# medivhna/TF_Face_Toolbox

Measured on NVIDIA B200. Metric: A-softmax head fwd+bwd samples/sec at C=85,742 D=512, 1/2/4/8 B200, higher is better.
Workload: dtype bf16

## Files before the change

### tf_face_toolbox_b200/csrc/asm_api.cu

```cuda
#include <math.h>
#include <stdio.h>
#include <stdlib.h>
#include <string.h>

#include <new>
#include <vector>

#include "../../include/asoftmax_b200.h"
#include "asm_kernels.cuh"

using namespace asmh;

struct asm_head {
  asm_config cfg;
  int device = 0;
  int num_sms = 148;
  int Cp = 0;
  int NT = 0;
  char* ws = nullptr;
  size_t ws_bytes = 0;
  Step st{};
  size_t dx_part_capacity = 0;
  UmmaMaps maps{};
  int maps_B = -1;
// ... 42 lines not shown
  if (c->D <= 0 || c->D % 16 != 0) return false;
  if (c->C_total <= 0 || c->C_local <= 0 || c->class_offset < 0) return false;
  if ((long long)c->class_offset + c->C_local > c->C_total) return false;
  if (c->B_max <= 0 || c->m < 1 || c->m > 4) return false;
  if (c->mode != ASM_MODE_FP32 && c->mode != ASM_MODE_BF16) return false;
  if (c->mode == ASM_MODE_BF16 && c->D % 64 != 0) return false;
  if (c->world < 1 || c->rank < 0 || c->rank >= c->world) return false;
  if (c->nccl_comm != nullptr) return false;
  return true;
}

bool use_x3(const asm_config& c) {
  if (c.mode != ASM_MODE_FP32 || c.D % 64 != 0) return false;
  const char* e = getenv("ASM_FP32_SIMT");
  return !(e && atoi(e) != 0);
}
bool use_tc(const asm_config& c) { return c.mode == ASM_MODE_BF16 || use_x3(c); }

Layout make_layout(const asm_config& c, int num_sms) {
  Layout L{};
  const bool tc = use_tc(c);
  const size_t planes = use_x3(c) ? 3 : 1;
  const size_t B = c.B_max, D = c.D;
  L.Cp = (int)align_up(c.C_local, 256);
  L.NT = (L.Cp + 127) / 128;
  if (L.NT < 2 * num_sms) L.NT = 2 * num_sms;
  L.MT = 2 * (int)((B + 127) / 128);
  if (L.MT < 4 * (int)((B + 255) / 256)) L.MT = 4 * (int)((B + 255) / 256);
  const int ks_simt = simt_dx_splits(c.B_max, c.D, L.Cp);
  const int ks_umma = umma_dx_splits(c.B_max, c.D, L.Cp, num_sms, 1);
  const int ks_one = tc ? umma_dx_splits(128, c.D, L.Cp, num_sms, 1)
                        : simt_dx_splits(128, c.D, L.Cp);
  const size_t cap_full = (size_t)(tc ? ks_umma : ks_simt) * B * D;
  const size_t cap_one = (size_t)ks_one * (B < 128 ? B : 128) * D;
  L.dx_capacity = cap_full > cap_one ? cap_full : cap_one;
  size_t off = 0;
  auto take = [&](size_t bytes) { size_t o = off; off = align_up(off + bytes, 256); return o; };
  L.ylocal = take(B * 4);
  L.flags = take(256);
  L.n = take(B * 4);
  L.inv_n = take(B * 4);
  L.inv_c = take((size_t)L.Cp * 4);
  L.margin = take(kMarginRecordFloats * 4);
  L.tgt_s = take(B * 4);
  L.tgt_f = take(B * 4);
  L.part = take(B * (size_t)L.NT * 8);
  L.stats_local = take(3 * B * 4);
  L.lse = take(B * 4);
  L.negoff = take(B * 4);
  L.gtarget = take(B * 4);
  L.rcoef = take(B * 4);
  L.rowloss = take(B * 4);
  L.counter = take(256);
  L.wsq_part = take(((size_t)L.Cp / 32 + 16) * 4);
  L.wsq_ticket = take(256);
  L.q_part = take((size_t)L.MT * L.Cp * 4);
  L.G = take(align_up(B, 64) * (size_t)L.Cp * (c.mode == ASM_MODE_BF16 ? 2 : 4));
  L.dx_part = take(L.dx_capacity * 4);
  if (tc) {
    L.Xb = take(planes * B * D * 2);
    L.Wb = take(planes * D * (size_t)L.Cp * 2);
  } else {
    L.Xs = take(B * D * 4);
  }
  if (c.world > 1) {
    L.Xg = take(B * D * 4);
    L.step_dev = take(256);
  }
  L.total = off;
  return L;
}

int fail(asm_head* h, int code, const char* fmt, const char* detail) {
  char* dst = h ? h->err : g_create_err;
  snprintf(dst, 512, fmt, detail ? detail : "");
  return code;
}

#define CU_TRY(h, expr)                                                         \
  do {                                                                          \
    cudaError_t e__ = (expr);                                                   \
    if (e__ != cudaSuccess) return fail(h, ASM_ERR_CUDA, #expr ": %s", cudaGetErrorString(e__)); \
  } while (0)

void mark(asm_head* h, const char* name, cudaStream_t stream, bool phase_start = true) {
  h->launches += 1;
  if (h->phase_profiling && !phase_start) return;
  if (h->profiling && h->n_marks < asm_head::kMaxMarks) {
    cudaEventRecord(h->ev[h->n_marks], stream);
    h->mark_name[h->n_marks] = name;
    h->n_marks += 1;
  }
}
void mark_end(asm_head* h, cudaStream_t stream) {
  if (h->profiling) cudaEventRecord(h->ev[h->n_marks], stream);
}

int check_launch(asm_head* h, const char* what) {
  cudaError_t e = cudaGetLastError();
  if (e != cudaSuccess) {
    snprintf(h->err, 512, "%s: %s", what, cudaGetErrorString(e));
    return ASM_ERR_CUDA;
  }
  return ASM_OK;
}

bool split_active(const asm_head* h) {
// ... 195 lines not shown
    return fail(nullptr, ASM_ERR_CUDA, "cudaGetDevice failed%s", "");
  cudaDeviceGetAttribute(&major, cudaDevAttrComputeCapabilityMajor, dev);
  cudaDeviceGetAttribute(&sms, cudaDevAttrMultiProcessorCount, dev);
  if (major != 10)
    return fail(nullptr, ASM_ERR_NO_DEVICE, "device is not sm_100 (Blackwell B200) %s", "");
  asm_head* h = new (std::nothrow) asm_head();
  if (!h) return fail(nullptr, ASM_ERR_ALLOC, "host allocation failed%s", "");
  h->cfg = *cfg;
  h->device = dev;
  h->num_sms = sms > 0 ? sms : 148;
  h->err[0] = 0;
  const char* e;
  if ((e = getenv("ASM_UMMA_MN_LBO"))) h->tune.mn_lbo = (uint32_t)atoi(e);
  if ((e = getenv("ASM_UMMA_MN_SBO"))) h->tune.mn_sbo = (uint32_t)atoi(e);
  if ((e = getenv("ASM_UMMA_MN_KSTEP"))) h->tune.mn_kstep = (uint32_t)atoi(e);
  if ((e = getenv("ASM_UMMA_DEBUG")) && atoi(e) != 0) {
#ifdef ASM_BRINGUP
    h->tune.debug_flags = (uint32_t)atoi(e);
#else
    delete h;
    return fail(nullptr, ASM_ERR_INVALID_ARG,
                "ASM_UMMA_DEBUG is set but this library was built without -DASM_BRINGUP%s", "");
#endif
  }
  if ((e = getenv("ASM_L2_ORDER"))) h->tune.l2_order = atoi(e) != 0;
  if ((e = getenv("ASM_DW_TMA"))) h->tune.dw_tma = atoi(e) != 0;
  if ((e = getenv("ASM_L2_HINTS"))) h->tune.l2_hints = (uint32_t)atoi(e);
  if ((e = getenv("ASM_UMMA_CG"))) h->tune.cg_mask = (uint32_t)atoi(e);
  if ((e = getenv("ASM_UMMA_BN"))) h->tune.bn = (uint32_t)atoi(e);
  if ((e = getenv("ASM_NO_OVERLAP")) && atoi(e)) h->overlap = false;
  h->dw_pairs = (h->num_sms / 2) * 42 / 74;
  if ((e = getenv("ASM_DW_PAIRS"))) h->dw_pairs = atoi(e);
  if (h->dw_pairs < 0 || h->dw_pairs >= h->num_sms / 2) h->dw_pairs = 0;
  if ((e = getenv("ASM_PDL"))) h->pdl = atoi(e) != 0;
  if ((e = getenv("ASM_DEFER_LOSS"))) h->defer_loss = atoi(e) != 0;
  if ((e = getenv("ASM_OPT_STREAM"))) h->opt_stream = atoi(e) != 0;
  if (cudaStreamCreateWithFlags(&h->side, cudaStreamNonBlocking) != cudaSuccess ||
      cudaEventCreateWithFlags(&h->ev_fork, cudaEventDisableTiming) != cudaSuccess ||
      cudaEventCreateWithFlags(&h->ev_join, cudaEventDisableTiming) != cudaSuccess) {
    cudaGetLastError();
    h->side = nullptr;
  }
  if ((e = getenv("ASM_L2_PERSIST_MB"))) h->l2_persist_bytes = (size_t)atoi(e) << 20;
  const Layout L = make_layout(*cfg, h->num_sms);
  cudaError_t ce = cudaMalloc(&h->ws, L.total);
  if (ce != cudaSuccess) {
    fail(nullptr, ASM_ERR_ALLOC, "cudaMalloc(workspace): %s", cudaGetErrorString(ce));
    delete h;
    return ASM_ERR_ALLOC;
  }
  h->ws_bytes = L.total;
  cudaMemset(h->ws, 0, L.total);
  h->tc = use_tc(*cfg);
  if (h->tc) {
    ce = umma_configure();
    if (ce != cudaSuccess) {
      fail(nullptr, ASM_ERR_CUDA, "cudaFuncSetAttribute(smem): %s", cudaGetErrorString(ce));
      cudaFree(h->ws);
      delete h;
      return ASM_ERR_CUDA;
    }
  }
  Step& s = h->st;
  s.D = cfg->D;
  s.C = cfg->C_local;
  s.Cp = L.Cp;
  s.C_total = cfg->C_total;
  s.class_offset = cfg->class_offset;
  s.m = cfg->m;
  s.mode = cfg->mode;
  s.x3 = use_x3(*cfg) ? 1 : 0;
  char* w = h->ws;
  s.ylocal = (int*)(w + L.ylocal);
  s.flags = (int*)(w + L.flags);
  s.n = (float*)(w + L.n);
  s.inv_n = (float*)(w + L.inv_n);
  s.inv_c = (float*)(w + L.inv_c);
  s.tgt_s = (float*)(w + L.tgt_s);
  s.tgt_f = (float*)(w + L.tgt_f);
  s.part = (float2*)(w + L.part);
  s.stats_local = (float*)(w + L.stats_local);
  s.lse = (float*)(w + L.lse);
  s.negoff = (float*)(w + L.negoff);
  s.gtarget = (float*)(w + L.gtarget);
  s.rcoef = (float*)(w + L.rcoef);
  s.rowloss = (float*)(w + L.rowloss);
  s.counter = (unsigned int*)(w + L.counter);
  s.q_part = (float*)(w + L.q_part);
  s.wsq_part = (float*)(w + L.wsq_part);
  s.wsq_ticket = (unsigned int*)(w + L.wsq_ticket);
  s.gscale = 1.0f;
  s.wd_g = 0.0f;
  s.reg_scale = 0.0f;
  s.reg_out = nullptr;
  s.G = (void*)(w + L.G);
  s.dx_part = (float*)(w + L.dx_part);
  h->dx_part_capacity = L.dx_capacity;
  if (h->tc) {
    s.Xb = (__nv_bfloat16*)(w + L.Xb);
    s.Wb = (__nv_bfloat16*)(w + L.Wb);
  } else {
    s.Xs = (float*)(w + L.Xs);
  }
  s.mg.kind = 0;
  if (cfg->world > 1) {
    h->Xg = (float*)(w + L.Xg);
// ... 290 lines not shown
```

### tf_face_toolbox_b200/csrc/asm_kernels.cuh

```cuda
#pragma once
#include <cuda.h>
#include <cuda_bf16.h>
#include <cuda_runtime.h>
#include <stdint.h>

#include "asm_common.cuh"

namespace asmh {

struct OptParams {
  int kind;
  float lr;
  float mu, b1, b2, eps, wd;
};
__host__ __device__ inline void opt_apply(const OptParams& o, float grad, float& w, float& s0,
                                          float& s1) {
  const float g = grad + o.wd * w;
  if (o.kind == 1) {
    s0 = o.mu * s0 + g;
    w -= o.lr * s0;
  } else {
    s0 = o.b1 * s0 + (1.0f - o.b1) * g;
    s1 = o.b2 * s1 + (1.0f - o.b2) * g * g;
#ifdef __CUDA_ARCH__
// ... 71 lines not shown
  int B, D, C, Cp, C_total, class_offset, m, mode;
  float lambda, invB;
  const float* lambda_dev;
  float gscale;
  float wd_g;
  float reg_scale;
  float* reg_out;
  float* wsq_part;
  unsigned int* wsq_ticket;
  const float* X;
  int x_bf16;
  const float* W;
  float* logits;
  float* dX;
  float* dW;
  float* loss;
  int* ylocal;
  int* flags;
  float* n;
  float* inv_n;
  float* inv_c;
  float* tgt_s;
  float* tgt_f;
  float2* part;
  int NT;
  float* stats_local;
  float* lse;
  float* negoff;
  float* gtarget;
  float* rcoef;
  float* rowloss;
  unsigned int* counter;
  float* q_part;
  int MT;
  void* G;
  int Bp;
  float* dx_part;
  int KS;
  __nv_bfloat16* Xb;
  __nv_bfloat16* Wb;
  int x3;
  OptParams opt;
  float* Wmut;
  float* opt_s0;
  float* opt_s1;
  int l2_hints;
  int pdl;
  int defer_loss;
  Margin mg;
  float* Xs;
};

void launch_prep(const Step& s, const void* labels, int label_bytes, cudaStream_t st, const P2P* p = nullptr);
void launch_combine_p2p(const Step& s, const P2P& p, cudaStream_t st);
void launch_dx_finish_p2p(const Step& s, const P2P& p, cudaStream_t st);
void launch_combine_local(const Step& s, cudaStream_t st);
void launch_combine_global(const Step& s, const float* stats_all, int n_shards, cudaStream_t st);
void launch_combine_fused(const Step& s, cudaStream_t st);
void launch_dx_finish(const Step& s, cudaStream_t st);
void launch_opt_stream(const Step& s, const float* dW, cudaStream_t st);

void p2p_preload_kernels();
void prep_preload_kernels();
void simt_preload_kernels();

void launch_simt_forward(const Step& s, cudaStream_t st);
void launch_simt_bwdg(const Step& s, cudaStream_t st);
void launch_simt_dw(const Step& s, cudaStream_t st);
void launch_simt_dx(const Step& s, cudaStream_t st);
int simt_forward_tiles(int C);
int simt_dx_splits(int B, int D, int Cp);

struct UmmaMaps {
  CUtensorMap xb_k, xb_k256, xb_mn, wb_mn, wb_mn32, wb_k, wb_k128, g_k, g_mn, g_st, g_st32, wb_box;
  CUtensorMap dw_even, dw_odd;
  CUtensorMap dx_st;
  int dx_ok;
  const void* dw_ptr;
  int dw_ok;
};
struct UmmaTuning {
  uint32_t mn_lbo, mn_sbo, mn_kstep;
  uint32_t cg_mask;
  uint32_t debug_flags;
  uint32_t bn;
  uint32_t l2_order;
  uint32_t dw_tma;
  uint32_t side_by_side;
  uint32_t l2_hints;
};
struct UmmaArgs {
  int mt, nt, ks, kb_total, kb_per;
  int nseg, kb_seg;
  int segA[6], segB[6];
  uint64_t desc_hi_k, desc_hi_mn;
  uint32_t kstep_mn;
  uint32_t debug_flags;
  int rev;
  int kstride;
  int dw_tma;
  int dx_tma;
  int dw_shift;
  int store_evict_first;
};
cudaError_t umma_configure();
bool umma_build_maps(UmmaMaps* m, const Step& s);
// ... 17 lines not shown
```

### tf_face_toolbox_b200/csrc/asm_prep.cu

```cuda
#include <stdlib.h>

#include "asm_common.cuh"
#include "asm_kernels.cuh"
#include "asm_p2p.cuh"
#include "asm_rows.cuh"

namespace asmh {

__device__ __forceinline__ void prep_row_tail(const Step& s, int row, float acc, long long y) {
  const float nn = sqrtf(acc);
  s.n[row] = nn;
  s.inv_n[row] = nn > 0.f ? 1.0f / nn : 0.f;
  const long long yl = y - s.class_offset;
  s.ylocal[row] = (y < 0 || y >= s.C_total) ? -2 : ((yl >= 0 && yl < s.C) ? (int)yl : -1);
  s.tgt_s[row] = 0.f;
  s.tgt_f[row] = 0.f;
}

template <int PL>
__device__ __forceinline__ void prep_row_scaled(const Step& s, const char* x, char* xg, int esz, bool gather,
                                                int row, long long y) {
  const int tx = threadIdx.x & 31;
  const float4* x4 = reinterpret_cast<const float4*>(x);
  const int n16 = s.D * esz / 16;
  const int epp = 16 / esz;
  auto sq16 = [&](const float4& v) {
    if (esz == 2) {
      const __nv_bfloat162* h2 = reinterpret_cast<const __nv_bfloat162*>(&v);
      float a = 0.f;
#pragma unroll
      for (int q = 0; q < 4; ++q) {
        const float l = __low2float(h2[q]), h = __high2float(h2[q]);
        a = fmaf(l, l, a);
        a = fmaf(h, h, a);
      }
      return a;
    }
    return fmaf(v.x, v.x, fmaf(v.y, v.y, fmaf(v.z, v.z, v.w * v.w)));
  };
  float4 v[4];
  float acc = 0.f;
  for (int i0 = 0; i0 < n16; i0 += 128) {
#pragma unroll
    for (int u = 0; u < 4; ++u) {
      const int i = i0 + u * 32 + tx;
      v[u] = i < n16 ? (gather ? __ldcv(x4 + i) : __ldg(x4 + i)) : make_float4(0.f, 0.f, 0.f, 0.f);
    }
#pragma unroll
    for (int u = 0; u < 4; ++u) {
      const int i = i0 + u * 32 + tx;
      if (i < n16) {
        if (gather) reinterpret_cast<float4*>(xg)[i] = v[u];
        acc += sq16(v[u]);
      }
    }
  }
  acc = warp_sum(acc);
  const float nn = sqrtf(acc);
  const float sc = nn > 0.f ? s.mg.s / nn : 0.f;
  auto put = [&](int d, float e) {
    const float u = e * sc;
    if (PL > 0) {
      __nv_bfloat16* dst = s.Xb + (size_t)row * PL * s.D + d;
      float r = u;
#pragma unroll
      for (int p2 = 0; p2 < PL; ++p2) {
        const __nv_bfloat16 hv = __float2bfloat16_rn(r);
        dst[(size_t)p2 * s.D] = hv;
        r -= __bfloat162float(hv);
      }
    } else {
      s.Xs[(size_t)row * s.D + d] = u;
    }
  };
  auto put16 = [&](int e0, const float4& w) {
    if (esz == 2) {
      const __nv_bfloat162* h2 = reinterpret_cast<const __nv_bfloat162*>(&w);
#pragma unroll
      for (int q = 0; q < 4; ++q) {
        put(e0 + 2 * q, __low2float(h2[q]));
        put(e0 + 2 * q + 1, __high2float(h2[q]));
      }
    } else {
      put(e0, w.x); put(e0 + 1, w.y); put(e0 + 2, w.z); put(e0 + 3, w.w);
    }
  };
  const float4* again = gather ? reinterpret_cast<const float4*>(xg) : x4;
  for (int i0 = 0; i0 < n16; i0 += 128) {
#pragma unroll
    for (int u = 0; u < 4; ++u) {
      const int i = i0 + u * 32 + tx;
      if (i < n16) put16(i * epp, n16 <= 128 ? v[u] : again[i]);
    }
  }
  if (tx == 0) prep_row_tail(s, row, acc, y);
}

template <bool VEC2, int PL, int TX, int TY, int U, bool ADD>
__device__ __forceinline__ void prep_block(const Step& s, const void* labels, int label_bytes,
                                           int nwb, int npub, const P2P& p, const int vblock,
                                           float (*red)[2 * TX]) {
  static_assert(TX * TY == 256, "256 threads");
  const int tid = threadIdx.x;
  if (vblock < npub) {
    const unsigned cur = p2p_current_step(p);
    float4* xs = reinterpret_cast<float4*>(p.x(p.rank, cur & 1));
    int* ys = p.y(p.rank, cur & 1);
    const size_t n4 = (size_t)p.b_local * p.D * (s.x_bf16 ? 2 : 4) / 16;
    for (size_t i = vblock * (size_t)256 + tid; i < n4; i += (size_t)npub * 256)
      xs[i] = __ldg(reinterpret_cast<const float4*>(p.x_local) + i);
    for (int i = vblock * 256 + tid; i < p.b_local; i += npub * 256)
      ys[i] = p.y_bytes == 8 ? (int)reinterpret_cast<const long long*>(p.y_local)[i]
                             : reinterpret_cast<const int*>(p.y_local)[i];
    if (block_ticket(p.tickets + 0, (unsigned)npub) == (unsigned)npub - 1 && tid == 0)
      p2p_publish(p, 0, cur);
    return;
  }
  const int bid = vblock - npub;
  if (bid < nwb) {
    const int tx = tid % TX, ty = tid / TX;
    const int j0 = (bid * TX + tx) * 2;
    float a0 = 0.f, a1 = 0.f;
    if (j0 < s.Cp) {
      const bool v0 = j0 < s.C, v1 = j0 + 1 < s.C;
      const float* w = s.W + j0;
      constexpr bool BF16 = PL > 0;
      __nv_bfloat16* wb = BF16 ? s.Wb + (size_t)(j0 >> 6) * s.D * 64 + (j0 & 63) : nullptr;
      const size_t plane = (size_t)s.D * s.Cp;
      for (int d0 = ty; d0 < s.D; d0 += TY * U) {
        float x0[U], x1[U];
#pragma unroll
        for (int u = 0; u < U; ++u) {
          const int d = d0 + TY * u;
          x0[u] = 0.f; x1[u] = 0.f;
          if (d < s.D) {
            if (VEC2) {
              if (v1) {
                const float2* wp = reinterpret_cast<const float2*>(w + (size_t)d * s.C);
                const float2 v = s.l2_hints ? __ldcs(wp) : __ldg(wp);
                x0[u] = v.x; x1[u] = v.y;
              } else if (v0) {
                x0[u] = __ldg(w + (size_t)d * s.C);
              }
            } else {
              if (v0) x0[u] = __ldg(w + (size_t)d * s.C);
              if (v1) x1[u] = __ldg(w + (size_t)d * s.C + 1);
            }
          }
        }
#pragma unroll
        for (int u = 0; u < U; ++u) {
          const int d = d0 + TY * u;
          a0 = fmaf(x0[u], x0[u], a0);
          a1 = fmaf(x1[u], x1[u], a1);
          if (BF16 && d < s.D) {
            __nv_bfloat162* dst = reinterpret_cast<__nv_bfloat162*>(wb + (size_t)d * 64);
            float r0 = x0[u], r1 = x1[u];
#pragma unroll
            for (int p = 0; p < PL; ++p) {
              const __nv_bfloat162 hv = __floats2bfloat162_rn(r0, r1);
              dst[(size_t)p * (plane / 2)] = hv;
              r0 -= __low2float(hv);
              r1 -= __high2float(hv);
            }
          }
        }
      }
    }
    red[ty][tx * 2] = a0;
    red[ty][tx * 2 + 1] = a1;
    __syncthreads();
    for (int t = tid; t < 2 * TX; t += 256) {
      float acc = 0.f;
#pragma unroll
      for (int r = 0; r < TY; ++r) acc += red[r][t];
      const int j = bid * 2 * TX + t;
      if (j < s.Cp) s.inv_c[j] = (j < s.C && acc > 0.f) ? rsqrtf(acc) : 0.f;
      if (s.reg_out) red[0][t] = j < s.C ? acc : 0.f;
    }
    if (s.reg_out) {
      __syncthreads();
      if (tid == 0) {
        float tot = 0.f;
        for (int t = 0; t < 2 * TX; ++t) tot += red[0][t];
        s.wsq_part[bid] = tot;
      }
      if (block_ticket(s.wsq_ticket, (unsigned)nwb) == (unsigned)nwb - 1) {
        __shared__ float wred[256];
        float acc = 0.f;
        for (int i = tid; i < nwb; i += 256) acc += __ldcg(s.wsq_part + i);
        wred[tid] = acc;
        __syncthreads();
        for (int o = 128; o > 0; o >>= 1) {
          if (tid < o) wred[tid] += wred[tid + o];
          __syncthreads();
        }
        if (tid == 0) *s.reg_out = s.reg_scale * wred[0];
      }
    }
  } else {
    const int tx = tid & 31;
    const int row = (bid - nwb) * 8 + (tid >> 5);
    if (row >= s.B) return;
    const int esz = s.x_bf16 ? 2 : 4;
    const char* x = reinterpret_cast<const char*>(s.X) + (size_t)row * s.D * esz;
    char* xg = nullptr;
    long long y;
    if (npub > 0) {
      const unsigned cur = p2p_current_step(p);
      const int src = row / p.b_local, lr = row - src * p.b_local;
      if (tx == 0) p2p_wait(p, 0, src, cur);
      __syncwarp();
      x = reinterpret_cast<const char*>(p.x(src, cur & 1)) + (size_t)lr * s.D * esz;
      xg = reinterpret_cast<char*>(p.Xg) + (size_t)row * s.D * esz;
      y = (long long)__ldcv(p.y(src, cur & 1) + lr);
    } else {
      y = label_bytes == 8 ? reinterpret_cast<const long long*>(labels)[row]
                           : (long long)reinterpret_cast<const int*>(labels)[row];
    }
    if (ADD) {
      prep_row_scaled<PL>(s, x, xg, esz, npub > 0, row, y);
      return;
    }
    float acc = 0.f;
    auto emit = [&](int d, float v) {
      acc = fmaf(v, v, acc);
      if (PL > 0) {
        __nv_bfloat16* dst = s.Xb + (size_t)row * PL * s.D + d;
        float r = v;
#pragma unroll
        for (int p2 = 0; p2 < PL; ++p2) {
          const __nv_bfloat16 hv = __float2bfloat16_rn(r);
          dst[(size_t)p2 * s.D] = hv;
          r -= __bfloat162float(hv);
        }
      }
    };
    auto emit16 = [&](int e0, const float4& v) {
      if (s.x_bf16) {
        const __nv_bfloat162* h2 = reinterpret_cast<const __nv_bfloat162*>(&v);
#pragma unroll
        for (int q = 0; q < 4; ++q) {
          emit(e0 + 2 * q, __low2float(h2[q]));
          emit(e0 + 2 * q + 1, __high2float(h2[q]));
        }
      } else {
        emit(e0, v.x); emit(e0 + 1, v.y); emit(e0 + 2, v.z); emit(e0 + 3, v.w);
      }
    };
    {
      const float4* x4 = reinterpret_cast<const float4*>(x);
      const int n16 = s.D * esz / 16;
      const int epp = 16 / esz;
      for (int i0 = 0; i0 < n16; i0 += 128) {
        float4 v[4];
#pragma unroll
        for (int u = 0; u < 4; ++u) {
          const int i = i0 + u * 32 + tx;
          v[u] = i < n16 ? (npub > 0 ? __ldcv(x4 + i) : __ldg(x4 + i)) : make_float4(0.f, 0.f, 0.f, 0.f);
        }
#pragma unroll
        for (int u = 0; u < 4; ++u) {
          const int i = i0 + u * 32 + tx;
          if (i < n16) {
            if (npub > 0) reinterpret_cast<float4*>(xg)[i] = v[u];
            emit16(i * epp, v[u]);
          }
        }
      }
    }
    acc = warp_sum(acc);
    if (tx == 0) prep_row_tail(s, row, acc, y);
  }
}

template <bool VEC2, int PL, int TX, int TY, int U, bool ADD>
__global__ void __launch_bounds__(256) prep_kernel(Step s, const void* labels, int label_bytes,
                                                   int nwb, int npub, P2P p) {
  pdl_trigger();
  __shared__ float red[TY][2 * TX];
  if (blockIdx.x == 0 && threadIdx.x == 0) *const_cast<Margin*>(margin_record(s.tgt_s)) = s.mg;
  prep_block<VEC2, PL, TX, TY, U, ADD>(s, labels, label_bytes, nwb, npub, p, (int)blockIdx.x, red);
}

template <int TX, int TY, int U, bool ADD>
static void launch_prep_t(const Step& s, const void* labels, int label_bytes, cudaStream_t st, const P2P* p) {
  const int nwb = (s.Cp + 2 * TX - 1) / (2 * TX);
  const int nxb = (s.B + 7) / 8;
  int npub = 0;
  P2P pp{};
  if (p != nullptr && p->world > 1) {
    pp = *p;
    npub = (int)(((size_t)p->b_local * p->D / 4 + 2047) / 2048);
    if (npub < 1) npub = 1;
    if (npub > 32) npub = 32;
  }
  const bool vec2 = (s.C % 2 == 0) && ((reinterpret_cast<uintptr_t>(s.W) & 7) == 0);
  dim3 grd(npub + nwb + nxb);
  if (s.x3) {
    if (vec2) prep_kernel<true, 3, TX, TY, U, ADD><<<grd, 256, 0, st>>>(s, labels, label_bytes, nwb, npub, pp);
    else prep_kernel<false, 3, TX, TY, U, ADD><<<grd, 256, 0, st>>>(s, labels, label_bytes, nwb, npub, pp);
  } else if (s.mode == 1) {
    if (vec2) prep_kernel<true, 1, TX, TY, U, ADD><<<grd, 256, 0, st>>>(s, labels, label_bytes, nwb, npub, pp);
    else prep_kernel<false, 1, TX, TY, U, ADD><<<grd, 256, 0, st>>>(s, labels, label_bytes, nwb, npub, pp);
  } else {
    if (vec2) prep_kernel<true, 0, TX, TY, U, ADD><<<grd, 256, 0, st>>>(s, labels, label_bytes, nwb, npub, pp);
    else prep_kernel<false, 0, TX, TY, U, ADD><<<grd, 256, 0, st>>>(s, labels, label_bytes, nwb, npub, pp);
  }
}

template <int TX, int TY, int U>
static void launch_prep_t(const Step& s, const void* labels, int label_bytes, cudaStream_t st, const P2P* p) {
  if (s.mg.kind != 0) launch_prep_t<TX, TY, U, true>(s, labels, label_bytes, st, p);
  else launch_prep_t<TX, TY, U, false>(s, labels, label_bytes, st, p);
}

void launch_prep(const Step& s, const void* labels, int label_bytes, cudaStream_t st, const P2P* p) {
  static int shape = -1, small_auto = -1;
  if (shape < 0) {
    const char* e = getenv("ASM_PREP_SHAPE");
    shape = e ? atoi(e) : 0;
    e = getenv("ASM_PREP_AUTO");
    small_auto = (e && atoi(e) != 0) ? 1 : 0;
  }
  if (shape == 0 && small_auto && s.Cp <= 32768) {
    launch_prep_t<16, 16, 8>(s, labels, label_bytes, st, p);
    return;
  }
  if (shape == 1) launch_prep_t<32, 8, 16>(s, labels, label_bytes, st, p);
  else if (shape == 2) launch_prep_t<16, 16, 8>(s, labels, label_bytes, st, p);
  else if (shape == 3) launch_prep_t<128, 2, 16>(s, labels, label_bytes, st, p);
  else launch_prep_t<32, 8, 4>(s, labels, label_bytes, st, p);
}

__global__ void __launch_bounds__(256) combine_local_kernel(Step s) {
  pdl_trigger();
  pdl_wait();
  const int row = blockIdx.x * 8 + (threadIdx.x >> 5);
  const int lane = threadIdx.x & 31;
  if (row >= s.B) return;
  float m = -INFINITY, z = 0.f;
  const float2* p = s.part + (size_t)row * s.NT;
  for (int t = lane; t < s.NT; t += 32) {
    const float2 v = p[t];
    ms_combine(m, z, v.x, v.y);
  }
#pragma unroll
  for (int o = 16; o > 0; o >>= 1) {
    const float m2 = __shfl_xor_sync(0xffffffffu, m, o);
    const float z2 = __shfl_xor_sync(0xffffffffu, z, o);
    ms_combine(m, z, m2, z2);
  }
  if (lane == 0) {
    float* st = s.stats_local;
    st[row] = m;
    st[s.B + row] = z;
    st[2 * s.B + row] = s.ylocal[row] >= 0 ? s.tgt_f[row] : 0.f;
  }
}

void launch_combine_local(const Step& s, cudaStream_t st) {
  launch_pdl(combine_local_kernel, dim3((s.B + 7) / 8), dim3(256), 0, st, s.pdl != 0, 1, s);
}

template <bool FUSED>
__global__ void __launch_bounds__(256) combine_kernel(Step s, const float* stats_all, int n_shards) {
  __shared__ float red[256];
  __shared__ bool is_last;
  pdl_trigger();
  pdl_wait();
  const int row = blockIdx.x * 8 + (threadIdx.x >> 5);
  const int lane = threadIdx.x & 31;
  if (row < s.B) {
    float m = -INFINITY, z = 0.f, fy = 0.f;
    const int yl_row = s.ylocal[row];
    const float tgt_f_row = s.tgt_f[row], tgt_s_row = s.tgt_s[row], inv_n_row = s.inv_n[row];
    if (FUSED) {
      const float2* p = s.part + (size_t)row * s.NT;
      for (int t = lane; t < s.NT; t += 32) {
        const float2 v = p[t];
        ms_combine(m, z, v.x, v.y);
      }
    } else {
      for (int g = lane; g < n_shards; g += 32) {
        const float* sg = stats_all + (size_t)g * 3 * s.B;
// ... 84 lines not shown
      g[0] = dW[i]; w[0] = W[i]; a[0] = s0[i]; b[0] = op.kind == 2 ? s1[i] : 0.f;
    }
#pragma unroll
    for (int v = 0; v < V; ++v) opt_apply(op, g[v], w[v], a[v], b[v]);
    if (V == 4) {
      *reinterpret_cast<float4*>(W + i) = make_float4(w[0], w[1], w[2], w[3]);
      *reinterpret_cast<float4*>(s0 + i) = make_float4(a[0], a[1], a[2], a[3]);
      if (op.kind == 2) *reinterpret_cast<float4*>(s1 + i) = make_float4(b[0], b[1], b[2], b[3]);
    } else {
      W[i] = w[0]; s0[i] = a[0];
      if (op.kind == 2) s1[i] = b[0];
    }
  }
}

void launch_opt_stream(const Step& s, const float* dW, cudaStream_t st) {
  const size_t n = (size_t)s.D * s.C;
  const uintptr_t al = reinterpret_cast<uintptr_t>(dW) | reinterpret_cast<uintptr_t>(s.Wmut) |
                       reinterpret_cast<uintptr_t>(s.opt_s0) | reinterpret_cast<uintptr_t>(s.opt_s1);
  if (n % 4 == 0 && (al & 15) == 0) {
    size_t blocks = (n / 4 + 255) / 256;
    if (blocks > 148 * 16) blocks = 148 * 16;
    launch_pdl(opt_stream_kernel<4>, dim3((unsigned)blocks), dim3(256), 0, st, false, 1, dW, s.Wmut, s.opt_s0,
               s.opt_s1, n, s.opt);
  } else {
    size_t blocks = (n + 255) / 256;
    if (blocks > 148 * 16) blocks = 148 * 16;
    launch_pdl(opt_stream_kernel<1>, dim3((unsigned)blocks), dim3(256), 0, st, false, 1, dW, s.Wmut, s.opt_s0,
               s.opt_s1, n, s.opt);
  }
}

template <int TX, int TY, int U, bool ADD>
static void preload_prep_t() {
  cudaFuncAttributes a;
  cudaFuncGetAttributes(&a, prep_kernel<true, 3, TX, TY, U, ADD>);
  cudaFuncGetAttributes(&a, prep_kernel<false, 3, TX, TY, U, ADD>);
  cudaFuncGetAttributes(&a, prep_kernel<true, 1, TX, TY, U, ADD>);
  cudaFuncGetAttributes(&a, prep_kernel<false, 1, TX, TY, U, ADD>);
  cudaFuncGetAttributes(&a, prep_kernel<true, 0, TX, TY, U, ADD>);
  cudaFuncGetAttributes(&a, prep_kernel<false, 0, TX, TY, U, ADD>);
}
template <int TX, int TY, int U>
static void preload_prep_t() {
  preload_prep_t<TX, TY, U, false>();
  preload_prep_t<TX, TY, U, true>();
}
void prep_preload_kernels() {
  preload_prep_t<16, 16, 8>();
  preload_prep_t<32, 8, 16>();
  preload_prep_t<128, 2, 16>();
  preload_prep_t<32, 8, 4>();
  cudaFuncAttributes a;
  cudaFuncGetAttributes(&a, combine_local_kernel);
  cudaFuncGetAttributes(&a, combine_kernel<true>);
  cudaFuncGetAttributes(&a, combine_kernel<false>);
  cudaFuncGetAttributes(&a, dx_finish_kernel<0>);
  cudaFuncGetAttributes(&a, dx_finish_margin_kernel);
  cudaFuncGetAttributes(&a, opt_stream_kernel<4>);
  cudaFuncGetAttributes(&a, opt_stream_kernel<1>);
}

}
```

### tf_face_toolbox_b200/csrc/asm_umma.cuh

```cuda
#pragma once
#include <cuda.h>
#include <cuda_runtime.h>
#include <stdint.h>
#include <stdio.h>

namespace asmh {
namespace ptx {

__device__ __forceinline__ uint32_t smem_u32(const void* p) {
  return static_cast<uint32_t>(__cvta_generic_to_shared(p));
}

__device__ __forceinline__ bool elect_one() {
  uint32_t pred;
  asm volatile(
      "{\n\t.reg .pred p;\n\t"
      "elect.sync _|p, 0xffffffff;\n\t"
      "selp.u32 %0, 1, 0, p;\n\t}\n"
      : "=r"(pred));
  return pred != 0;
}

__device__ __forceinline__ void mbar_init(uint64_t* bar, uint32_t count) {
  asm volatile("mbarrier.init.shared::cta.b64 [%0], %1;" ::"r"(smem_u32(bar)), "r"(count));
// ... 1 lines not shown
__device__ __forceinline__ void fence_barrier_init() {
  asm volatile("fence.mbarrier_init.release.cluster;" ::: "memory");
}
__device__ __forceinline__ void fence_proxy_async() {
  asm volatile("fence.proxy.async.shared::cta;" ::: "memory");
}
__device__ __forceinline__ void mbar_expect_tx(uint64_t* bar, uint32_t bytes) {
  asm volatile("mbarrier.arrive.expect_tx.shared::cta.b64 _, [%0], %1;" ::"r"(smem_u32(bar)),
               "r"(bytes)
               : "memory");
}
__device__ __forceinline__ void mbar_arrive(uint64_t* bar) {
  asm volatile("mbarrier.arrive.shared::cta.b64 _, [%0];" ::"r"(smem_u32(bar)) : "memory");
}
__device__ __forceinline__ bool mbar_try_wait(uint32_t addr, uint32_t parity) {
  uint32_t ok;
  asm volatile(
      "{\n\t.reg .pred p;\n\t"
      "mbarrier.try_wait.parity.shared::cta.b64 p, [%1], %2;\n\t"
      "selp.u32 %0, 1, 0, p;\n\t}\n"
      : "=r"(ok)
      : "r"(addr), "r"(parity)
      : "memory");
  return ok != 0;
}
__device__ __forceinline__ void mbar_wait(uint64_t* bar, uint32_t parity) {
  const uint32_t addr = smem_u32(bar);
  if (mbar_try_wait(addr, parity)) return;
  const long long t0 = clock64();
  while (!mbar_try_wait(addr, parity)) {
    if (clock64() - t0 > 4000000000ll) {
      printf("asoftmax_b200: mbarrier timeout block %d thread %d smem 0x%x parity %u\n",
             (int)blockIdx.x, (int)threadIdx.x, addr, parity);
      __trap();
    }
  }
}

__device__ __forceinline__ void prefetch_l2(const void* p) {
  asm volatile("prefetch.global.L2 [%0];" ::"l"(p));
}
__device__ __forceinline__ void prefetch_tmap(const CUtensorMap* m) {
  asm volatile("prefetch.tensormap [%0];" ::"l"(reinterpret_cast<uint64_t>(m)) : "memory");
}
__device__ __forceinline__ void tma_load_2d(void* smem_dst, const CUtensorMap* m, uint64_t* bar,
                                            int32_t c0, int32_t c1) {
  asm volatile(
      "cp.async.bulk.tensor.2d.shared::cluster.global.mbarrier::complete_tx::bytes"
      " [%0], [%1, {%3, %4}], [%2];" ::"r"(smem_u32(smem_dst)),
      "l"(reinterpret_cast<uint64_t>(m)), "r"(smem_u32(bar)), "r"(c0), "r"(c1)
      : "memory");
}

__device__ __forceinline__ void tma_store_2d(const CUtensorMap* m, const void* smem_src,
                                             int32_t c0, int32_t c1) {
  asm volatile(
      "cp.async.bulk.tensor.2d.global.shared::cta.bulk_group [%0, {%2, %3}], [%1];" ::"l"(
          reinterpret_cast<uint64_t>(m)),
      "r"(smem_u32(smem_src)), "r"(c0), "r"(c1)
      : "memory");
}
__device__ __forceinline__ void tma_store_3d(const CUtensorMap* m, const void* smem_src, int32_t c0,
                                             int32_t c1, int32_t c2) {
  asm volatile(
      "cp.async.bulk.tensor.3d.global.shared::cta.bulk_group [%0, {%2, %3, %4}], [%1];" ::"l"(
          reinterpret_cast<uint64_t>(m)),
      "r"(smem_u32(smem_src)), "r"(c0), "r"(c1), "r"(c2)
      : "memory");
}
__device__ __forceinline__ void tma_store_2d_hint(const CUtensorMap* m, const void* smem_src,
                                                  int32_t c0, int32_t c1, uint64_t policy) {
  asm volatile(
      "cp.async.bulk.tensor.2d.global.shared::cta.bulk_group.L2::cache_hint [%0, {%2, %3}], [%1], %4;" ::"l"(
          reinterpret_cast<uint64_t>(m)),
      "r"(smem_u32(smem_src)), "r"(c0), "r"(c1), "l"(policy)
      : "memory");
}
__device__ __forceinline__ uint64_t policy_evict_first() {
  uint64_t p;
  asm volatile("createpolicy.fractional.L2::evict_first.b64 %0, 1.0;" : "=l"(p));
  return p;
}
__device__ __forceinline__ void bulk_commit() {
  asm volatile("cp.async.bulk.commit_group;" ::: "memory");
}
__device__ __forceinline__ void bulk_wait_read0() {
  asm volatile("cp.async.bulk.wait_group.read 0;" ::: "memory");
}
__device__ __forceinline__ void bulk_wait_read1() {
  asm volatile("cp.async.bulk.wait_group.read 1;" ::: "memory");
}
__device__ __forceinline__ void bulk_wait0() {
  asm volatile("cp.async.bulk.wait_group 0;" ::: "memory");
}

__device__ __forceinline__ void tmem_alloc(uint32_t* smem_result, uint32_t ncols) {
  asm volatile("tcgen05.alloc.cta_group::1.sync.aligned.shared::cta.b32 [%0], %1;" ::"r"(
                   smem_u32(smem_result)),
               "r"(ncols)
               : "memory");
}
__device__ __forceinline__ void tmem_relinquish() {
  asm volatile("tcgen05.relinquish_alloc_permit.cta_group::1.sync.aligned;" ::: "memory");
}
__device__ __forceinline__ void tmem_dealloc(uint32_t taddr, uint32_t ncols) {
  asm volatile("tcgen05.dealloc.cta_group::1.sync.aligned.b32 %0, %1;" ::"r"(taddr), "r"(ncols)
// ... 123 lines not shown
```

Measured before the change: 2.238 million.

## Add warp-specialized bulk-copy pipelined prep kernel for single-device weight prep

Adds a new prep kernel that streams weight rows through a multi-stage shared-memory ring filled by 1D bulk async copies from a producer warp. Consumer warps compute per-class squared norms and bf16 split planes, while separate warps process input rows concurrently. It is used for single-device runs in the default shape instead of the old prep launch, and wsq_part becomes per-class rather than per-warp. The aim is to hide global-load latency and raise bandwidth on the large weight read. In exchange it adds smem configuration, ragged edge handling and a last-block reduction.

Result: slower. 1.315 million (median of 6 runs) (-41.3%).

```diff
diff --git a/tf_face_toolbox_b200/csrc/asm_api.cu b/tf_face_toolbox_b200/csrc/asm_api.cu
--- a/tf_face_toolbox_b200/csrc/asm_api.cu
+++ b/tf_face_toolbox_b200/csrc/asm_api.cu
@@ -118,7 +118,7 @@
   L.rcoef = take(B * 4);
   L.rowloss = take(B * 4);
   L.counter = take(256);
-  L.wsq_part = take(((size_t)L.Cp / 32 + 16) * 4);
+  L.wsq_part = take(((size_t)L.Cp + 16) * 4);
   L.wsq_ticket = take(256);
   L.q_part = take((size_t)L.MT * L.Cp * 4);
   L.G = take(align_up(B, 64) * (size_t)L.Cp * (c.mode == ASM_MODE_BF16 ? 2 : 4));
@@ -420,6 +420,13 @@
   h->ws_bytes = L.total;
   cudaMemset(h->ws, 0, L.total);
   h->tc = use_tc(*cfg);
+  ce = prep_configure();
+  if (ce != cudaSuccess) {
+    fail(nullptr, ASM_ERR_CUDA, "cudaFuncSetAttribute(prep smem): %s", cudaGetErrorString(ce));
+    cudaFree(h->ws);
+    delete h;
+    return ASM_ERR_CUDA;
+  }
   if (h->tc) {
     ce = umma_configure();
     if (ce != cudaSuccess) {
diff --git a/tf_face_toolbox_b200/csrc/asm_kernels.cuh b/tf_face_toolbox_b200/csrc/asm_kernels.cuh
--- a/tf_face_toolbox_b200/csrc/asm_kernels.cuh
+++ b/tf_face_toolbox_b200/csrc/asm_kernels.cuh
@@ -147,6 +147,7 @@
 };
 
 void launch_prep(const Step& s, const void* labels, int label_bytes, cudaStream_t st, const P2P* p = nullptr);
+cudaError_t prep_configure();
 void launch_combine_p2p(const Step& s, const P2P& p, cudaStream_t st);
 void launch_dx_finish_p2p(const Step& s, const P2P& p, cudaStream_t st);
 void launch_combine_local(const Step& s, cudaStream_t st);
diff --git a/tf_face_toolbox_b200/csrc/asm_prep.cu b/tf_face_toolbox_b200/csrc/asm_prep.cu
--- a/tf_face_toolbox_b200/csrc/asm_prep.cu
+++ b/tf_face_toolbox_b200/csrc/asm_prep.cu
@@ -4,6 +4,7 @@
 #include "asm_kernels.cuh"
 #include "asm_p2p.cuh"
 #include "asm_rows.cuh"
+#include "asm_umma.cuh"
 
 namespace asmh {
 
@@ -93,6 +94,81 @@
       if (i < n16) put16(i * epp, n16 <= 128 ? v[u] : again[i]);
     }
   }
+  if (tx == 0) prep_row_tail(s, row, acc, y);
+}
+
+template <int PL, bool ADD>
+__device__ __forceinline__ void prep_x_row(const Step& s, const void* labels, int label_bytes, bool gather,
+                                           const P2P& p, int row) {
+  const int tx = threadIdx.x & 31;
+  const int esz = s.x_bf16 ? 2 : 4;
+  const char* x = reinterpret_cast<const char*>(s.X) + (size_t)row * s.D * esz;
+  char* xg = nullptr;
+  long long y;
+  if (gather) {
+    const unsigned cur = p2p_current_step(p);
+    const int src = row / p.b_local, lr = row - src * p.b_local;
+    if (tx == 0) p2p_wait(p, 0, src, cur);
+    __syncwarp();
+    x = reinterpret_cast<const char*>(p.x(src, cur & 1)) + (size_t)lr * s.D * esz;
+    xg = reinterpret_cast<char*>(p.Xg) + (size_t)row * s.D * esz;
+    y = (long long)__ldcv(p.y(src, cur & 1) + lr);
+  } else {
+    y = label_bytes == 8 ? reinterpret_cast<const long long*>(labels)[row]
+                         : (long long)reinterpret_cast<const int*>(labels)[row];
+  }
+  if (ADD) {
+    prep_row_scaled<PL>(s, x, xg, esz, gather, row, y);
+    return;
+  }
+  float acc = 0.f;
+  auto emit = [&](int d, float v) {
+    acc = fmaf(v, v, acc);
+    if (PL > 0) {
+      __nv_bfloat16* dst = s.Xb + (size_t)row * PL * s.D + d;
+      float r = v;
+#pragma unroll
+      for (int p2 = 0; p2 < PL; ++p2) {
+        const __nv_bfloat16 hv = __float2bfloat16_rn(r);
+        dst[(size_t)p2 * s.D] = hv;
+        r -= __bfloat162float(hv);
+      }
+    }
+  };
+  auto emit16 = [&](int e0, const float4& v) {
+    if (s.x_bf16) {
+      const __nv_bfloat162* h2 = reinterpret_cast<const __nv_bfloat162*>(&v);
+#pragma unroll
+      for (int q = 0; q < 4; ++q) {
+        emit(e0 + 2 * q, __low2float(h2[q]));
+        emit(e0 + 2 * q + 1, __high2float(h2[q]));
+      }
+    } else {
+      emit(e0, v.x); emit(e0 + 1, v.y); emit(e0 + 2, v.z); emit(e0 + 3, v.w);
+    }
+  };
+  {
+    const float4* x4 = reinterpret_cast<const float4*>(x);
+    const int n16 = s.D * esz / 16;
+    const int epp = 16 / esz;
+    for (int i0 = 0; i0 < n16; i0 += 128) {
+      float4 v[4];
+#pragma unroll
+      for (int u = 0; u < 4; ++u) {
+        const int i = i0 + u * 32 + tx;
+        v[u] = i < n16 ? (gather ? __ldcv(x4 + i) : __ldg(x4 + i)) : make_float4(0.f, 0.f, 0.f, 0.f);
+      }
+#pragma unroll
+      for (int u = 0; u < 4; ++u) {
+        const int i = i0 + u * 32 + tx;
+        if (i < n16) {
+          if (gather) reinterpret_cast<float4*>(xg)[i] = v[u];
+          emit16(i * epp, v[u]);
+        }
+      }
+    }
+  }
+  acc = warp_sum(acc);
   if (tx == 0) prep_row_tail(s, row, acc, y);
 }
 
@@ -199,78 +275,9 @@
       }
     }
   } else {
-    const int tx = tid & 31;
     const int row = (bid - nwb) * 8 + (tid >> 5);
     if (row >= s.B) return;
-    const int esz = s.x_bf16 ? 2 : 4;
-    const char* x = reinterpret_cast<const char*>(s.X) + (size_t)row * s.D * esz;
-    char* xg = nullptr;
-    long long y;
-    if (npub > 0) {
-      const unsigned cur = p2p_current_step(p);
-      const int src = row / p.b_local, lr = row - src * p.b_local;
-      if (tx == 0) p2p_wait(p, 0, src, cur);
-      __syncwarp();
-      x = reinterpret_cast<const char*>(p.x(src, cur & 1)) + (size_t)lr * s.D * esz;
-      xg = reinterpret_cast<char*>(p.Xg) + (size_t)row * s.D * esz;
-      y = (long long)__ldcv(p.y(src, cur & 1) + lr);
-    } else {
-      y = label_bytes == 8 ? reinterpret_cast<const long long*>(labels)[row]
-                           : (long long)reinterpret_cast<const int*>(labels)[row];
-    }
-    if (ADD) {
-      prep_row_scaled<PL>(s, x, xg, esz, npub > 0, row, y);
-      return;
-    }
-    float acc = 0.f;
-    auto emit = [&](int d, float v) {
-      acc = fmaf(v, v, acc);
-      if (PL > 0) {
-        __nv_bfloat16* dst = s.Xb + (size_t)row * PL * s.D + d;
-        float r = v;
-#pragma unroll
-        for (int p2 = 0; p2 < PL; ++p2) {
-          const __nv_bfloat16 hv = __float2bfloat16_rn(r);
-          dst[(size_t)p2 * s.D] = hv;
-          r -= __bfloat162float(hv);
-        }
-      }
-    };
-    auto emit16 = [&](int e0, const float4& v) {
-      if (s.x_bf16) {
-        const __nv_bfloat162* h2 = reinterpret_cast<const __nv_bfloat162*>(&v);
-#pragma unroll
-        for (int q = 0; q < 4; ++q) {
-          emit(e0 + 2 * q, __low2float(h2[q]));
-          emit(e0 + 2 * q + 1, __high2float(h2[q]));
-        }
-      } else {
-        emit(e0, v.x); emit(e0 + 1, v.y); emit(e0 + 2, v.z); emit(e0 + 3, v.w);
-      }
-    };
-    {
-      const float4* x4 = reinterpret_cast<const float4*>(x);
-      const int n16 = s.D * esz / 16;
-      const int epp = 16 / esz;
-      for (int i0 = 0; i0 < n16; i0 += 128) {
-        float4 v[4];
-#pragma unroll
-        for (int u = 0; u < 4; ++u) {
-          const int i = i0 + u * 32 + tx;
-          v[u] = i < n16 ? (npub > 0 ? __ldcv(x4 + i) : __ldg(x4 + i)) : make_float4(0.f, 0.f, 0.f, 0.f);
-        }
-#pragma unroll
-        for (int u = 0; u < 4; ++u) {
-          const int i = i0 + u * 32 + tx;
-          if (i < n16) {
-            if (npub > 0) reinterpret_cast<float4*>(xg)[i] = v[u];
-            emit16(i * epp, v[u]);
-          }
-        }
-      }
-    }
-    acc = warp_sum(acc);
-    if (tx == 0) prep_row_tail(s, row, acc, y);
+    prep_x_row<PL, ADD>(s, labels, label_bytes, npub > 0, p, row);
   }
 }
 
@@ -315,6 +322,206 @@
   else launch_prep_t<TX, TY, U, false>(s, labels, label_bytes, st, p);
 }
 
+namespace stream_prep {
+constexpr int kRows = 8;
+constexpr int kCW = 512;
+constexpr int kRowPitch = kCW * 4 + 16;
+constexpr int kStageBytes = kRows * kRowPitch;
+constexpr int kStages = 6;
+constexpr int kConsumerWarps = 8, kXWarps = 4;
+constexpr int kThreads = 32 * (1 + kConsumerWarps + kXWarps);
+constexpr int kSmem = kStages * kStageBytes + 2 * kStages * 8;
+}
+
+template <int PL, bool ADD>
+__global__ void __launch_bounds__(stream_prep::kThreads, 2)
+    prep_stream_kernel(Step s, const void* labels, int label_bytes) {
+  using namespace stream_prep;
+  pdl_trigger();
+  extern __shared__ __align__(16) unsigned char sm[];
+  uint64_t* full = reinterpret_cast<uint64_t*>(sm + kStages * kStageBytes);
+  uint64_t* empty = full + kStages;
+  const int tid = threadIdx.x, warp = tid >> 5;
+  if (blockIdx.x == 0 && tid == 0) *const_cast<Margin*>(margin_record(s.tgt_s)) = s.mg;
+  if (tid == 0) {
+    for (int i = 0; i < kStages; ++i) {
+      ptx::mbar_init(&full[i], 1);
+      ptx::mbar_init(&empty[i], kConsumerWarps);
+    }
+    ptx::fence_barrier_init();
+  }
+  __syncthreads();
+
+  const int units = s.Cp / 8;
+  const int lo = (int)((long long)units * blockIdx.x / gridDim.x) * 8;
+  const int hi = (int)((long long)units * (blockIdx.x + 1) / gridDim.x) * 8;
+  const int nchunk = (hi - lo + kCW - 1) / kCW;
+  const int nst = s.D / kRows;
+
+  if (warp == 0) {
+    if ((tid & 31) == 0) {
+      const char* wbase = reinterpret_cast<const char*>(s.W);
+      const char* wend = wbase + (size_t)s.D * s.C * 4;
+      const char* wa = reinterpret_cast<const char*>((reinterpret_cast<uintptr_t>(wbase) + 15) & ~(uintptr_t)15);
+      const char* wz = reinterpret_cast<const char*>(reinterpret_cast<uintptr_t>(wend) & ~(uintptr_t)15);
+      const uint64_t pol = ptx::policy_evict_first();
+      const bool hint = s.l2_hints != 0;
+      int it = 0;
+      for (int k = 0; k < nchunk; ++k) {
+        const int c0 = lo + k * kCW;
+        const int vc = min(min(c0 + kCW, hi), s.C) - c0;
+        for (int st = 0; st < nst; ++st, ++it) {
+          const int slot = it % kStages;
+          if (it >= kStages) ptx::mbar_wait(&empty[slot], ((it / kStages) & 1) ^ 1);
+          unsigned char* buf = sm + slot * kStageBytes;
+          uint32_t bytes = 0;
+          bool ragged = false;
+          for (int i = 0; i < kRows && vc > 0; ++i) {
+            const char* g0 = wbase + ((size_t)(st * kRows + i) * s.C + c0) * 4;
+            const char* g1 = g0 + (size_t)vc * 4;
+            const char* a = reinterpret_cast<const char*>(reinterpret_cast<uintptr_t>(g0) & ~(uintptr_t)15);
+            const char* b = reinterpret_cast<const char*>((reinterpret_cast<uintptr_t>(g1) + 15) & ~(uintptr_t)15);
+            const char* ca = a < wa ? wa : a;
+            const char* cb = b > wz ? wz : b;
+            if (cb <= ca) ca = cb = g1;
+            unsigned char* row = buf + i * kRowPitch;
+            for (const char* g = g0; g < (ca < g1 ? ca : g1); g += 4) {
+              *reinterpret_cast<float*>(row + (g - a)) = __ldg(reinterpret_cast<const float*>(g));
+              ragged = true;
+            }
+            for (const char* g = cb > g0 ? cb : g0; g < g1; g += 4) {
+              *reinterpret_cast<float*>(row + (g - a)) = __ldg(reinterpret_cast<const float*>(g));
+              ragged = true;
+            }
+            if (cb > ca) ptx::bulk_load_1d(row + (ca - a), ca, (uint32_t)(cb - ca), &full[slot], hint, pol);
+            bytes += (uint32_t)(cb - ca);
+          }
+          if (ragged) ptx::fence_proxy_async();
+          ptx::mbar_expect_tx(&full[slot], bytes);
+        }
+      }
+    }
+  } else if (warp <= kConsumerWarps) {
+    const int ct = tid - 32;
+    float a0[kRows], a1[kRows];
+    int sh[kRows];
+#pragma unroll
+    for (int i = 0; i < kRows; ++i)
+      sh[i] = (int)((reinterpret_cast<uintptr_t>(s.W) + (size_t)i * s.C * 4) & 15);
+    const size_t plane = (size_t)s.D * s.Cp;
+    int it = 0;
+    for (int k = 0; k < nchunk; ++k) {
+      const int c0 = lo + k * kCW;
+      const int j = c0 + 2 * ct;
+      const bool act = j < min(c0 + kCW, hi);
+      const bool v0 = j < s.C, v1 = j + 1 < s.C;
+#pragma unroll
+      for (int i = 0; i < kRows; ++i) a0[i] = a1[i] = 0.f;
+      __nv_bfloat16* wb = PL > 0 ? s.Wb + (size_t)(j >> 6) * s.D * 64 + (j & 63) : nullptr;
+      for (int st = 0; st < nst; ++st, ++it) {
+        const int slot = it % kStages;
+        ptx::mbar_wait(&full[slot], (it / kStages) & 1);
+        if (act) {
+          const unsigned char* buf = sm + slot * kStageBytes + 8 * ct;
+#pragma unroll
+          for (int i = 0; i < kRows; ++i) {
+            const float* e = reinterpret_cast<const float*>(buf + i * kRowPitch + sh[i]);
+            const float x0 = v0 ? e[0] : 0.f, x1 = v1 ? e[1] : 0.f;
+            a0[i] = fmaf(x0, x0, a0[i]);
+            a1[i] = fmaf(x1, x1, a1[i]);
+            if (PL > 0) {
+              __nv_bfloat162* dst = reinterpret_cast<__nv_bfloat162*>(wb + (size_t)(st * kRows + i) * 64);
+              float r0 = x0, r1 = x1;
+#pragma unroll
+              for (int q = 0; q < PL; ++q) {
+                const __nv_bfloat162 hv = __floats2bfloat162_rn(r0, r1);
+                dst[(size_t)q * (plane / 2)] = hv;
+                r0 -= __low2float(hv);
+                r1 -= __high2float(hv);
+              }
+            }
+          }
+        }
+        __syncwarp();
+        if ((tid & 31) == 0) ptx::mbar_arrive(&empty[slot]);
+      }
+      if (act) {
+        float t0 = 0.f, t1 = 0.f;
+#pragma unroll
+        for (int i = 0; i < kRows; ++i) {
+          t0 += a0[i];
+          t1 += a1[i];
+        }
+        s.inv_c[j] = (v0 && t0 > 0.f) ? rsqrtf(t0) : 0.f;
+        s.inv_c[j + 1] = (v1 && t1 > 0.f) ? rsqrtf(t1) : 0.f;
+        if (s.reg_out) {
+          s.wsq_part[j] = v0 ? t0 : 0.f;
+          s.wsq_part[j + 1] = v1 ? t1 : 0.f;
+        }
+      }
+    }
+  } else {
+    for (int row = blockIdx.x * kXWarps + (warp - 1 - kConsumerWarps); row < s.B; row += gridDim.x * kXWarps)
+      prep_x_row<PL, ADD>(s, labels, label_bytes, false, P2P{}, row);
+  }
+  __syncwarp();
+
+  if (s.reg_out) {
+    if (block_ticket(s.wsq_ticket, gridDim.x) == gridDim.x - 1) {
+      __shared__ float wred[256];
+      const int nwb = s.Cp / 64;
+      if (tid < 256) {
+        float acc = 0.f;
+        for (int b = tid; b < nwb; b += 256) {
+          float tot = 0.f;
+          for (int t = 0; t < 64; ++t) tot += __ldcg(s.wsq_part + b * 64 + t);
+          acc += tot;
+        }
+        wred[tid] = acc;
+      }
+      __syncthreads();
+      for (int o = 128; o > 0; o >>= 1) {
+        if (tid < o) wred[tid] += wred[tid + o];
+        __syncthreads();
+      }
+      if (tid == 0) *s.reg_out = s.reg_scale * wred[0];
+    }
+  }
+}
+
+static int device_sms() {
+  static int sms[64];
+  int dev = 0;
+  cudaGetDevice(&dev);
+  if (dev < 0 || dev >= 64) dev = 0;
+  if (sms[dev] == 0 && cudaDeviceGetAttribute(&sms[dev], cudaDevAttrMultiProcessorCount, dev) != cudaSuccess)
+    sms[dev] = 148;
+  return sms[dev];
+}
+
+template <int PL, bool ADD>
+static void launch_prep_stream_t(const Step& s, const void* labels, int label_bytes, cudaStream_t st) {
+  prep_stream_kernel<PL, ADD><<<device_sms(), stream_prep::kThreads, stream_prep::kSmem, st>>>(s, labels, label_bytes);
+}
+
+cudaError_t prep_configure() {
+  const void* k[] = {(const void*)prep_stream_kernel<0, false>, (const void*)prep_stream_kernel<1, false>,
+                     (const void*)prep_stream_kernel<3, false>, (const void*)prep_stream_kernel<0, true>,
+                     (const void*)prep_stream_kernel<1, true>, (const void*)prep_stream_kernel<3, true>};
+  for (const void* f : k) {
+    const cudaError_t e = cudaFuncSetAttribute(f, cudaFuncAttributeMaxDynamicSharedMemorySize, stream_prep::kSmem);
+    if (e != cudaSuccess) return e;
+  }
+  return cudaSuccess;
+}
+
+template <bool ADD>
+static void launch_prep_stream(const Step& s, const void* labels, int label_bytes, cudaStream_t st) {
+  if (s.x3) launch_prep_stream_t<3, ADD>(s, labels, label_bytes, st);
+  else if (s.mode == 1) launch_prep_stream_t<1, ADD>(s, labels, label_bytes, st);
+  else launch_prep_stream_t<0, ADD>(s, labels, label_bytes, st);
+}
+
 void launch_prep(const Step& s, const void* labels, int label_bytes, cudaStream_t st, const P2P* p) {
   static int shape = -1, small_auto = -1;
   if (shape < 0) {
@@ -330,7 +537,9 @@
   if (shape == 1) launch_prep_t<32, 8, 16>(s, labels, label_bytes, st, p);
   else if (shape == 2) launch_prep_t<16, 16, 8>(s, labels, label_bytes, st, p);
   else if (shape == 3) launch_prep_t<128, 2, 16>(s, labels, label_bytes, st, p);
-  else launch_prep_t<32, 8, 4>(s, labels, label_bytes, st, p);
+  else if (p != nullptr && p->world > 1) launch_prep_t<32, 8, 4>(s, labels, label_bytes, st, p);
+  else if (s.mg.kind != 0) launch_prep_stream<true>(s, labels, label_bytes, st);
+  else launch_prep_stream<false>(s, labels, label_bytes, st);
 }
 
 __global__ void __launch_bounds__(256) combine_local_kernel(Step s) {
@@ -521,6 +730,12 @@
   preload_prep_t<128, 2, 16>();
   preload_prep_t<32, 8, 4>();
   cudaFuncAttributes a;
+  cudaFuncGetAttributes(&a, prep_stream_kernel<3, false>);
+  cudaFuncGetAttributes(&a, prep_stream_kernel<1, false>);
+  cudaFuncGetAttributes(&a, prep_stream_kernel<0, false>);
+  cudaFuncGetAttributes(&a, prep_stream_kernel<3, true>);
+  cudaFuncGetAttributes(&a, prep_stream_kernel<1, true>);
+  cudaFuncGetAttributes(&a, prep_stream_kernel<0, true>);
   cudaFuncGetAttributes(&a, combine_local_kernel);
   cudaFuncGetAttributes(&a, combine_kernel<true>);
   cudaFuncGetAttributes(&a, combine_kernel<false>);
diff --git a/tf_face_toolbox_b200/csrc/asm_umma.cuh b/tf_face_toolbox_b200/csrc/asm_umma.cuh
--- a/tf_face_toolbox_b200/csrc/asm_umma.cuh
+++ b/tf_face_toolbox_b200/csrc/asm_umma.cuh
@@ -77,6 +77,22 @@
       : "memory");
 }
 
+__device__ __forceinline__ void bulk_load_1d(void* smem_dst, const void* src, uint32_t bytes, uint64_t* bar,
+                                             bool hint, uint64_t policy) {
+  if (hint)
+    asm volatile(
+        "cp.async.bulk.shared::cluster.global.mbarrier::complete_tx::bytes.L2::cache_hint"
+        " [%0], [%1], %2, [%3], %4;" ::"r"(smem_u32(smem_dst)),
+        "l"(reinterpret_cast<uint64_t>(src)), "r"(bytes), "r"(smem_u32(bar)), "l"(policy)
+        : "memory");
+  else
+    asm volatile(
+        "cp.async.bulk.shared::cluster.global.mbarrier::complete_tx::bytes"
+        " [%0], [%1], %2, [%3];" ::"r"(smem_u32(smem_dst)),
+        "l"(reinterpret_cast<uint64_t>(src)), "r"(bytes), "r"(smem_u32(bar))
+        : "memory");
+}
+
 __device__ __forceinline__ void tma_store_2d(const CUtensorMap* m, const void* smem_src,
                                              int32_t c0, int32_t c1) {
   asm volatile(
```
